# foamdino/incubator-druid

Measured on AMD Instinct MI355X. Metric: filtered rows aggregated/sec, higher is better.
Workload: dtype int64/f64; 1 GPU; BASELINE configs[2]: GroupByV2 dimUniform x dimHyperUnique (3-byte ids, ~1 group/row) + longSum/doubleSum, 100M rows = 8 x 12.5M-row segments per MI355X; config=groupby, segments_per_gpu=8, compression=lz4, lz4_mode=hc, bitmap=concise, long_encoding=longs, parallelism=segments sharded over 1 GPU(s)

## Files before the change

### incubator-druid_amd/csrc/dg_engine.cpp

```cpp
#include <hip/hip_runtime.h>

#include <algorithm>
#include <atomic>
#include <chrono>
#include <thread>
#include <functional>
#include <cerrno>
#include <cmath>
#include <cstdarg>
#include <cstdio>
#include <cstdlib>
#include <cstring>
#include <queue>
#include <unordered_map>
#include <string>
#include <string_view>
#include <vector>

#include "dg_internal.h"

namespace dg {

static thread_local char g_err[1024] = "";
static thread_local uint64_t g_err_count = 0;
// ... 4002 lines not shown
  if (choice.max_groups > 0) max_groups = std::min(max_groups, choice.max_groups);
  if (key_bits < 62) max_groups = std::min<int64_t>(max_groups, (int64_t)1 << key_bits);
  HashTable tab{};
  const bool use_hash = choice.grouper == DG_GROUPER_HASH && !has_float_sum(plan) && key_bits <= 63 &&
                        hash_capacity(max_groups) <= ((int64_t)1 << 31);
  if (use_hash) {
    tab.capacity = hash_capacity(max_groups);
    tab.log2_capacity = bits_for(tab.capacity);
    tab.max_groups = max_groups;
    tab.keys = dev_take<uint64_t>(cs, (size_t)tab.capacity);
    tab.slots = dev_take<uint64_t>(cs, (size_t)tab.capacity * rec);
    tab.ctr = dev_take<unsigned long long>(cs, 4);
    if (!tab.keys || !tab.slots || !tab.ctr)
      return set_error(DG_ERR_OOM, "hash table of %lld slots x %d words", (long long)tab.capacity, rec + 1);
    if (!call_err(cs, st)) return set_error(DG_ERR_OOM, "error word");
  }
  uint32_t* h_n = host_take<uint32_t>(cs, 4);
  if (!h_n) return set_error(DG_ERR_OOM, "groupBy counters");
  DG_FLUSH(cs, st);
  phase_event(ctx->ev[3], st);
  auto all_rows_in = [&](int i) {
    if (gj[i].bitset || gj[i].multi) return false;
    if (gj[i].time.kind == VIEW_ABSENT) return true;
    const Column* tc = sv[i]->find("__time");
    if (!tc || !tc->data.time_col || tc->data.nblocks <= 0 || tc->data.min8.size() != (size_t)tc->data.nblocks ||
        tc->data.max8.size() != (size_t)tc->data.nblocks)
      return false;
    const int64_t lo = *std::min_element(tc->data.min8.begin(), tc->data.min8.end());
    const int64_t hi = *std::max_element(tc->data.max8.begin(), tc->data.max8.end());
    return lo >= gj[i].t_lo && hi < gj[i].t_hi;
  };
  bool rows_elems = !any_multi && !has_float_sum(plan) && !env_on("DG_GB_COUNT");
  for (int i = 0; i < n && rows_elems; ++i) rows_elems = !cur[i].any || all_rows_in(i);
  launch_gb_keygen(d_jobs, d_tile, ntiles, &sb, plan, st, any_multi, rows_elems ? total : -1);
  phase_event(ctx->ev[5], st);
  unsigned long long* h_ctr = nullptr;
  if (use_hash) {
    h_ctr = host_take<unsigned long long>(cs, 4);
    if (!h_ctr) return set_error(DG_ERR_OOM, "groupBy counters");
    launch_gb_hash_fill(tab, plan, st);
    if (side) DG_HIP(hipStreamWaitEvent(st, ctx->side_ev[2], 0));
    launch_gb_hash_insert(&sb, sb.cap, tab, plan, cs->d_err, st);
    phase_event(ctx->ev[6], st);
    DG_HIP(hipMemcpyAsync(h_ctr, tab.ctr, 32, hipMemcpyDeviceToHost, st));
    DG_HIP(hipMemcpyAsync(h_n, sb.n, 4, hipMemcpyDeviceToHost, st));
    rc = finish_call(cs, st);
    if (rc == DG_ERR_TABLE_FULL)
      return set_error(DG_ERR_TABLE_FULL, "groupBy hash table full: more than %lld groups (bufferGrouperMaxSize; %lld slots)",
                       (long long)tab.max_groups, (long long)tab.capacity);
    if (rc) return rc;
  } else {
    launch_radix_sort(&sb, key_bits, st);
    phase_event(ctx->ev[6], st);
  }
  DG_CHECK_INTERRUPT(intr);
  const int64_t cap = std::max<int64_t>(use_hash ? (int64_t)h_ctr[0] : sb.cap, 1);
  PendingResult res(new dg_result());
  res->ctx = ctx;
  res->ndims = nd;
  res->naggs = na;
  res->lay = lay;
  res->bucket0 = gb0;
  res->period = q->period_ms;
  if (gr.hb) res->bounds.assign(gr.hb, gr.hb + gr.nb + 1);
  res->universal = q->interval_start;
  res->kinds.assign(plan.kind, plan.kind + na);
  res->dicts = md;
  res->keys = static_cast<uint64_t*>(result_alloc(ctx, (size_t)cap * 8));
  res->slots = static_cast<uint64_t*>(result_alloc(ctx, (size_t)cap * rec * 8));
  res->cap = cap;
  if (!res->keys || !res->slots) return set_error(DG_ERR_OOM, "groupBy result of %lld records", (long long)cap);
  bool reduce_timed = false;
  if (use_hash) {
    const int64_t ngh = (int64_t)h_ctr[0];
    phase_event(ctx->ev[7], st);
    reduce_timed = true;
    if (ngh > 0) {
      SortBufs gsb;
      rc = sort_bufs(cs, ngh, 1, key_bits, 0, &gsb, tab.log2_capacity);
      if (rc) return rc;
      launch_gb_hash_collect(tab, &gsb, ngh, st);
      launch_radix_sort(&gsb, key_bits, st);
      launch_gb_hash_emit(&gsb, ngh, tab, plan, res->keys, res->slots, cap, st);
    }
    res->grouper.grouper = DG_GROUPER_HASH;
// ... 37 lines not shown
        DG_HIP(hipStreamSynchronize(st));
        DG_HIP(hipGetLastError());
      }
      result_free(ctx, res->keys);
      result_free(ctx, res->slots);
      res->keys = k2;
      res->slots = s2;
      res->cap = c2;
    } else {
      result_free(ctx, k2);
      result_free(ctx, s2);
    }
  }
  if (side) {
    float fs = 0;
    phase_elapsed(&fs, ctx->side_ev[1], ctx->side_ev[2]);
    m.decode_side_ms = fs;
  }
  for (int i = 0; i < n; ++i)
    if (cur[i].any) m.pre_filtered_rows += counts[i] ? (int64_t)*counts[i] : sv[i]->nrows;
  m.selected_rows = nsel;
  float f1 = 0, f2 = 0, f3 = 0, f4 = 0, f5 = 0, f6 = 0;
  phase_elapsed(&f1, ctx->ev[0], ctx->ev[1]);
  phase_elapsed(&f2, ctx->ev[1], ctx->ev[2]);
  phase_elapsed(&f3, ctx->ev[3], ctx->ev[4]);
  phase_elapsed(&f4, ctx->ev[3], ctx->ev[5]);
  phase_elapsed(&f5, ctx->ev[5], ctx->ev[6]);
  phase_elapsed(&f6, ctx->ev[6], ctx->ev[4]);
  m.bitmap_ms = f1;
  m.bitmap_bytes = cs->bitmap_bytes;
  m.decode_ms = f2;
  decode_metrics(db, db_side, &m, ctx->ev[0]);
  m.aggregate_ms = f3;
  m.keygen_ms = f4;
  m.sort_ms = f5;
  m.reduce_ms = f6;
  if (reduce_timed) {
    float fr = 0;
    phase_elapsed(&fr, ctx->ev[7], ctx->ev[4]);
    m.reduce_kernel_ms = fr;
  }
  m.sort_passes = key_bits > 0 ? (key_bits + 7) / 8 : 0;
  m.key_bits = key_bits;
  m.groups = ng;
  m.total_ms = ms_since(t0);
  if (metrics) *metrics = m;
  *out = res.release();
  return DG_OK;
}

int64_t dg_result_groups(const dg_result* r) { return r ? r->ngroups : -1; }

int dg_result_grouper_info(const dg_result* r, dg_grouper_info* out) {
  if (!r || !out) return set_error(DG_ERR_ARG, "null argument");
  *out = r->grouper;
  return DG_OK;
}

int dg_result_fetch_groups(dg_result* r, int64_t start, int64_t count, int64_t* bucket_time, int32_t* ids,
                           uint64_t* values) {
  if (!r || start < 0 || count < 0 || start + count > r->ngroups) return set_error(DG_ERR_ARG, "bad result range");
  if (count == 0) return DG_OK;
  CallGuard g(r->ctx);
  CallScratch* cs = g.cs;
  hipStream_t st = r->ctx->stream;
  const int nd = r->ndims, na = r->naggs;
  const int64_t per = (bucket_time ? 8 : 0) + (ids ? 4 * (int64_t)nd : 0) + (values ? 8 * (int64_t)na : 0);
// ... 1072 lines not shown
```

### incubator-druid_amd/csrc/dg_internal.h

```cpp
#pragma once

#include <hip/hip_runtime.h>
#include <stdint.h>
#include <string.h>

#include <algorithm>
#include <atomic>
#include <map>
#include <memory>
#include <mutex>
#include <string>
#include <vector>

#include "../../include/druidgpu.h"

namespace dg {

constexpr int kMaxAggs = 16;
constexpr int kBlockBytes = 65536;

enum Codec : int32_t { CODEC_LZF = 0x00, CODEC_LZ4 = 0x01, CODEC_UNCOMPRESSED = 0xFF, CODEC_NONE = 0xFE };

enum ViewKind : int32_t { VIEW_ABSENT = 0, VIEW_LONG = 1, VIEW_FLOAT = 2, VIEW_DOUBLE = 3, VIEW_IDS = 4 };

// ... 474 lines not shown
  int32_t dim_mode;
  const int32_t* rank;
  int32_t lo, hi;
  int32_t min_rank;
  int32_t pad;
};
constexpr int kSelBlock = 1024;
constexpr int kTopnOrderCap = 4096;
void launch_topn_select(const TopnSelJob* d_jobs, int njobs, int64_t max_card, int naggs, int metric, int metric_op,
                        int inverted, int threshold, hipStream_t s);

constexpr int kTileRows = 2048;

#ifndef DG_RS_DIGIT_BITS
#define DG_RS_DIGIT_BITS 8
#endif
constexpr int kMaxDigitBits = DG_RS_DIGIT_BITS;
constexpr int kMaxBins = 1 << kMaxDigitBits;
constexpr int kRsMaxPasses = 8;
constexpr int kSortTile = 4096;
#ifndef DG_RED_WAVES
#define DG_RED_WAVES 16
#endif
constexpr int kRedWaves = DG_RED_WAVES;
constexpr int kMaxCallSegs = 1024;
inline int sort_tiles(int64_t n) { return (int)std::max<int64_t>(1, (n + kSortTile - 1) / kSortTile); }
void launch_gb_count(const GbJob* d_jobs, const int32_t* d_tile_job, int ntiles, uint32_t* tile_cnt, uint32_t* total,
                     bool multi, hipStream_t s);
void launch_gb_count_total(const GbJob* d_jobs, const int32_t* d_tile_job, int ntiles, uint32_t* tile_cnt,
                           unsigned long long* total, hipStream_t s);
void launch_gb_keygen(const GbJob* d_jobs, const int32_t* d_tile_job, int ntiles, SortBufs* sb, AggPlan plan,
                      hipStream_t s, bool multi = false, int64_t all_rows = -1);
void launch_radix_sort(SortBufs* sb, int key_bits, hipStream_t s);
void launch_run_heads(SortBufs* sb, hipStream_t s);
void launch_run_mark(SortBufs* sb, uint32_t* head_pos, hipStream_t s);
void launch_gb_reduce(SortBufs* sb, AggPlan plan, uint64_t* out_keys, uint64_t* out_slots, int64_t cap,
                      uint32_t* head_pos, int64_t* carry_g, uint64_t* carry_slots, int64_t* open_g, hipStream_t s);
void launch_fsum_runs(const GbJob* d_jobs, int njobs, int ntiles, SortBufs* sb, AggPlan plan, int agg,
                      const uint32_t* head_pos, uint64_t* out_slots, int64_t cap, hipStream_t s, int desc = 0);
void launch_slots_finalize(uint64_t* slots, const uint32_t* n_ptr, int64_t cap, AggPlan plan, hipStream_t s);
void launch_soa_to_aos(const uint64_t* soa, int64_t cap, int64_t n, int rec, uint64_t* aos, hipStream_t s);
void launch_result_compact(const uint64_t* keys, const uint64_t* slots, int64_t cap, int64_t n, int rec, uint64_t* keys2,
                           uint64_t* slots2, hipStream_t s);
constexpr uint64_t kHashEmpty = ~0ull;
constexpr int32_t kErrTableFull = 8;
constexpr int kHashTile = 4096;
struct HashTable {
  uint64_t* keys;
  uint64_t* slots;
  int64_t capacity;
  int log2_capacity;
  int64_t max_groups;
  unsigned long long* ctr;
};
inline int64_t hash_capacity(int64_t max_groups) {
  int64_t c = 1;
  while (c * 7 < max_groups * 10) c <<= 1;
  return c;
}
struct GrouperChoice {
  int32_t grouper;
  int64_t max_groups;
};
inline GrouperChoice resolve_grouper(const dg_groupby_opts* opts, int32_t ctx_grouper, int64_t ctx_max_groups,
                                     const char* env) {
  GrouperChoice c{ctx_grouper, ctx_max_groups > 0 ? ctx_max_groups : 0};
// ... 47 lines not shown
```

### incubator-druid_amd/csrc/dg_sort.hip

```cpp
#include <hip/hip_runtime.h>
#include <cstring>

#include "dg_device.h"

namespace dg {

static bool zero_async(void* p, size_t n, hipStream_t s) {
  const hipError_t e = hipMemsetAsync(p, 0, n, s);
  if (e != hipSuccess) note_launch_error(e);
  return e == hipSuccess;
}

constexpr int kST = 256;
constexpr int kSPT = kSortTile / kST;
#ifndef DG_RS_TILE_MUL
#define DG_RS_TILE_MUL 1
#endif
#ifndef DG_RS_THREADS
#define DG_RS_THREADS 256
#endif
constexpr int kRsTile = kSortTile * DG_RS_TILE_MUL;
constexpr int kRsT = DG_RS_THREADS;
constexpr int kRsW = kRsT / 64;
constexpr int kRsSPT = kRsTile / kRsT;

template <int NT>
__device__ __forceinline__ uint64_t block_scan_u64(uint64_t v, uint64_t* total, uint64_t* s_tmp) {
  const int lane = threadIdx.x & 63, wave = threadIdx.x >> 6;
  uint64_t x = v;
#pragma unroll
  for (int o = 1; o < 64; o <<= 1) {
    const uint64_t y = __shfl_up(x, o, 64);
    if (lane >= o) x += y;
  }
// ... 25 lines not shown
    const int i = base + threadIdx.x;
    const uint32_t v = i < n ? a[i] : 0u;
    uint32_t t;
    const uint32_t ex = block_scan_u32<1024>(v, &t, s_tmp);
    if (i < n) a[i] = carry + ex;
    carry += t;
  }
  if (threadIdx.x == 0) *total = carry;
}

__device__ __forceinline__ size_t pay_at(int pw, size_t i, int a) { return i * (size_t)pw + (size_t)a; }

__device__ __forceinline__ int locate_seg(const uint32_t* s_base, int njobs, uint32_t ref) {
  int lo = 0, hi = njobs - 1;
  while (lo < hi) {
    const int mid = (lo + hi + 1) >> 1;
    if (s_base[mid] <= ref) lo = mid;
    else hi = mid - 1;
  }
  return lo;
}

__device__ __forceinline__ bool gb_select(const GbJob& j, int64_t r, int64_t* bucket) {
  if (j.bitset && !((j.bitset[r >> 5] >> (r & 31)) & 1u)) return false;
  *bucket = 0;
  if (j.time.kind != VIEW_ABSENT) {
    const int64_t t = load_time(j.time, r);
    if (t < j.t_lo || t >= j.t_hi) return false;
    if (j.period) *bucket = (bucket_coord(j.bounds, j.nbounds, t) - j.bucket0) / j.period;
  }
  return true;
}

__device__ __forceinline__ uint64_t gb_key(const GbJob& j, int64_t r, int64_t bucket) {
  uint64_t k = ((uint64_t)j.seg_slot << j.seg_shift) | ((uint64_t)bucket << j.bucket_shift);
  for (int d = 0; d < j.ndims; ++d) {
    uint32_t g;
    if (j.dims[d].kind == VIEW_IDS) {
      const uint32_t id = load_id(j.dims[d], r);
      g = j.remap[d] ? (uint32_t)j.remap[d][id] : id;
    } else {
      g = (uint32_t)j.null_gid[d];
    }
    k |= (uint64_t)g << j.dim_shift[d];
  }
  return k;
}

__device__ __forceinline__ uint32_t gb_fanout(const GbJob& j, int64_t r) {
  uint64_t n = 1;
  for (int d = 0; d < j.ndims; ++d)
    if (j.moff[d].kind != VIEW_ABSENT) {
      const uint32_t a = load_id(j.moff[d], r), b = load_id(j.moff[d], r + 1);
      n *= b > a ? (uint64_t)(b - a) : (j.skip_empty ? 0ull : 1ull);
      n = n > 0xFFFFFFFFull ? 0xFFFFFFFFull : n;
    }
  return (uint32_t)n;
}

__device__ __forceinline__ uint64_t gb_key_multi(const GbJob& j, int64_t r, int64_t bucket, uint32_t c) {
  uint64_t k = ((uint64_t)j.seg_slot << j.seg_shift) | ((uint64_t)bucket << j.bucket_shift);
  for (int d = j.ndims - 1; d >= 0; --d) {
    uint32_t g = (uint32_t)j.null_gid[d];
    if (j.moff[d].kind != VIEW_ABSENT) {
      const uint32_t a = load_id(j.moff[d], r), b = load_id(j.moff[d], r + 1);
      if (b > a) {
        const uint32_t m = b - a, i = c % m;
        c /= m;
        const uint32_t id = load_id(j.dims[d], (int64_t)a + i);
        g = j.remap[d] ? (uint32_t)j.remap[d][id] : id;
      }
    } else if (j.dims[d].kind == VIEW_IDS) {
      const uint32_t id = load_id(j.dims[d], r);
      g = j.remap[d] ? (uint32_t)j.remap[d][id] : id;
    }
    k |= (uint64_t)g << j.dim_shift[d];
  }
  return k;
}
// ... 23 lines not shown

__global__ __launch_bounds__(1024) void k_sum_u64(const uint32_t* __restrict__ a, int n, unsigned long long* __restrict__ total) {
  __shared__ unsigned long long s[16];
  unsigned long long c = 0;
  for (int i = threadIdx.x; i < n; i += 1024) c += a[i];
  for (int o = 32; o > 0; o >>= 1) c += __shfl_down(c, o, 64);
  if ((threadIdx.x & 63) == 0) s[threadIdx.x >> 6] = c;
  __syncthreads();
  if (threadIdx.x == 0) {
    unsigned long long t = 0;
    for (int w = 0; w < 16; ++w) t += s[w];
    *total = t;
  }
}

void launch_gb_count_total(const GbJob* d_jobs, const int32_t* d_tile_job, int ntiles, uint32_t* tile_cnt,
                           unsigned long long* total, hipStream_t s) {
  if (ntiles <= 0) {
    zero_async(total, 8, s);
    return;
  }
  hipLaunchKernelGGL(k_gb_count<true>, dim3(ntiles), dim3(256), 0, s, d_jobs, d_tile_job, tile_cnt);
  hipLaunchKernelGGL(k_sum_u64, dim3(1), dim3(1024), 0, s, tile_cnt, ntiles, total);
}

__device__ __forceinline__ uint32_t elem_ref(uint64_t w, const uint32_t* refs, int64_t i, int kshift) {
  return refs ? refs[i] : (uint32_t)(w & ((1ull << kshift) - 1ull));
}

template <bool MULTI>
__global__ __launch_bounds__(256) void k_gb_keygen(const GbJob* __restrict__ jobs, const int32_t* __restrict__ tile_job,
                                                   const uint32_t* __restrict__ offs, uint64_t* __restrict__ keys,
                                                   uint32_t* __restrict__ refs, int kshift, AggPlan plan,
                                                   uint64_t* __restrict__ payload, int pw, int rowref, int rows_elems) {
  __shared__ uint32_t s_tmp[4];
  const GbJob& j = jobs[tile_job[blockIdx.x]];
  const int64_t r0 = (int64_t)(blockIdx.x - j.tile_begin) * kTileRows;
  const int64_t r1 = min((int64_t)j.nrows, r0 + kTileRows);
  uint32_t base = rows_elems ? j.row_base + (uint32_t)r0 : offs[blockIdx.x];
  const uint32_t inplace = rowref ? j.inplace : 0u;
  const bool all_inplace = pw > 0 && inplace == (pw >= 32 ? 0xFFFFFFFFu : (1u << pw) - 1u);
  auto emit = [&](uint32_t idx, uint32_t ref, uint64_t key, auto&& val) {
    if (refs) {
      keys[idx] = key;
      refs[idx] = ref;
    } else {
      keys[idx] = (key << kshift) | ref;
    }
    if (all_inplace) return;
    if (pw == 2 && !inplace) {
      *reinterpret_cast<ulonglong2*>(payload + (size_t)ref * 2) = make_ulonglong2(val(0), val(1));
    } else {
      for (int a = 0; a < pw; ++a)
        if (!((inplace >> a) & 1u)) payload[pay_at(pw, ref, a)] = val(a);
    }
  };
  bool all_rows = !MULTI && !j.bitset;
  int64_t tbucket = 0;
  if (all_rows && j.time.kind != VIEW_ABSENT) {
    const int64_t tk = r0 >> j.time.log2_per;
    all_rows = (reinterpret_cast<uintptr_t>(j.time.blocks[tk]) & 1u) && tk == ((r1 - 1) >> j.time.log2_per);
    if (all_rows) all_rows = gb_select(j, r0, &tbucket);
  }
  if (all_rows) {
    bool direct = pw <= kMaxAggs;
    for (int d = 0; d < j.ndims; ++d)
      direct &= j.dims[d].kind != VIEW_IDS ||
                (!(j.dims[d].pad & kViewBigEndian) && (r0 >> j.dims[d].log2_per) == ((r1 - 1) >> j.dims[d].log2_per));
    for (int a = 0; a < pw; ++a)
      direct &= ((inplace >> a) & 1u) || j.vals[a].kind == VIEW_ABSENT ||
                (r0 >> j.vals[a].log2_per) == ((r1 - 1) >> j.vals[a].log2_per);
    if (direct) {
      constexpr int kB = kTileRows / 256;
      static_assert(kTileRows % 256 == 0, "whole batches per tile");
      uint64_t key[kB];
#pragma unroll
      for (int u = 0; u < kB; ++u) key[u] = ((uint64_t)j.seg_slot << j.seg_shift) | ((uint64_t)tbucket << j.bucket_shift);
      auto load_ids = [&](int d, uint32_t* id) {
        const ColView& v = j.dims[d];
        if (v.kind != VIEW_IDS) return;
        const int64_t blk = r0 >> v.log2_per;
        const uint8_t* bp = v.blocks[blk];
#pragma unroll
        for (int u = 0; u < kB; ++u) {
          const int64_t r = r0 + threadIdx.x + 256 * u;
          id[u] = 0;
          if (r < r1) {
            const uint32_t off = (uint32_t)(r - (blk << v.log2_per)) * (uint32_t)v.width;
            if (v.width == 3) {
              const uint32_t* w = reinterpret_cast<const uint32_t*>(bp + (off & ~3u));
              id[u] = __builtin_amdgcn_alignbyte(w[1], w[0], off & 3u) & 0xFFFFFFu;
            } else if (v.width == 1) {
              id[u] = bp[off];
            } else if (v.width == 2) {
              id[u] = *reinterpret_cast<const uint16_t*>(bp + off);
            } else {
              id[u] = *reinterpret_cast<const uint32_t*>(bp + off);
            }
          }
        }
      };
      auto merge_ids = [&](int d, uint32_t* id) {
        const int32_t* rm = j.remap[d];
        if (j.dims[d].kind != VIEW_IDS) {
#pragma unroll
          for (int u = 0; u < kB; ++u) key[u] |= (uint64_t)(uint32_t)j.null_gid[d] << j.dim_shift[d];
          return;
        }
#pragma unroll
        for (int u = 0; u < kB; ++u) key[u] |= (uint64_t)(rm ? (uint32_t)rm[id[u]] : id[u]) << j.dim_shift[d];
      };
      if (j.ndims == 2) {
        uint32_t id0[kB], id1[kB];
        load_ids(0, id0);
        load_ids(1, id1);
        merge_ids(0, id0);
        merge_ids(1, id1);
      } else {
        for (int d = 0; d < j.ndims; ++d) {
          uint32_t id[kB];
          load_ids(d, id);
          merge_ids(d, id);
        }
      }
#pragma unroll
      for (int u = 0; u < kB; ++u) {
        const int64_t r = r0 + threadIdx.x + 256 * u;
        if (r >= r1) continue;
        const uint32_t idx = base + (uint32_t)(r - r0);
        emit(idx, rowref ? j.row_base + (uint32_t)r : idx, key[u], [&](int a) -> uint64_t {
          const ColView& v = j.vals[a];
          if (!agg_row(j.agg_bits[a], r)) return identity_of(plan.op[a], plan.kind[a]);
          if (plan.kind[a] == DG_AGG_COUNT || v.kind == VIEW_ABSENT) return agg_input_at(plan.kind[a], v.kind, nullptr);
          const int64_t blk = r0 >> v.log2_per;
          return agg_input_at(plan.kind[a], v.kind, v.blocks[blk] + (size_t)(r - (blk << v.log2_per)) * (size_t)v.width);
        });
      }
      return;
    }
    for (int64_t r = r0 + threadIdx.x; r < r1; r += 256) {
      const uint32_t idx = base + (uint32_t)(r - r0);
      emit(idx, rowref ? j.row_base + (uint32_t)r : idx, gb_key(j, r, tbucket), [&](int a) { return agg_in(j, plan, a, r); });
    }
    return;
  }
  for (int64_t rb = r0; rb < r1; rb += 256) {
    const int64_t r = rb + threadIdx.x;
    int64_t b = 0;
    const bool sel = r < r1 && gb_select(j, r, &b);
    uint32_t tot;
    if (MULTI) {
      const uint32_t nf = sel ? gb_fanout(j, r) : 0u;
      const uint32_t ex = block_scan_u32<256>(nf, &tot, s_tmp);
      for (uint32_t e = 0; e < nf; ++e)
        emit(base + ex + e, base + ex + e, gb_key_multi(j, r, b, e), [&](int a) { return agg_in(j, plan, a, r); });
      base += tot;
      continue;
// ... 2 lines not shown
    if (sel)
      emit(base + ex, rowref ? j.row_base + (uint32_t)r : base + ex, gb_key(j, r, b),
           [&](int a) { return agg_in(j, plan, a, r); });
    base += tot;
  }
}

void launch_gb_count(const GbJob* d_jobs, const int32_t* d_tile_job, int ntiles, uint32_t* tile_cnt, uint32_t* total,
                     bool multi, hipStream_t s) {
  if (ntiles <= 0) {
    zero_async(total, 4, s);
    return;
  }
  if (multi) hipLaunchKernelGGL(k_gb_count<true>, dim3(ntiles), dim3(256), 0, s, d_jobs, d_tile_job, tile_cnt);
  else hipLaunchKernelGGL(k_gb_count<false>, dim3(ntiles), dim3(256), 0, s, d_jobs, d_tile_job, tile_cnt);
  hipLaunchKernelGGL(k_scan_u32, dim3(1), dim3(1024), 0, s, tile_cnt, ntiles, total);
}

void launch_gb_keygen(const GbJob* d_jobs, const int32_t* d_tile_job, int ntiles, SortBufs* sb, AggPlan plan,
                      hipStream_t s, bool multi, int64_t all_rows) {
  if (ntiles <= 0) {
    zero_async(sb->n, 4, s);
    return;
  }
  const bool rows_elems = !multi && all_rows >= 0;
  if (rows_elems) {
    const hipError_t e = hipMemsetD32Async(reinterpret_cast<hipDeviceptr_t>(sb->n), (int)(uint32_t)all_rows, 1, s);
    if (e != hipSuccess) note_launch_error(e);
  } else {
    launch_gb_count(d_jobs, d_tile_job, ntiles, sb->tile_cnt, sb->n, multi, s);
  }
  if (multi)
    hipLaunchKernelGGL(k_gb_keygen<true>, dim3(ntiles), dim3(256), 0, s, d_jobs, d_tile_job, sb->tile_cnt,
                       sb->keys[sb->cur], sb->refs[sb->cur], sb->ref_bits, plan, sb->payload, sb->pw, 0, 0);
  else
    hipLaunchKernelGGL(k_gb_keygen<false>, dim3(ntiles), dim3(256), 0, s, d_jobs, d_tile_job, sb->tile_cnt,
                       sb->keys[sb->cur], sb->refs[sb->cur], sb->ref_bits, plan, sb->payload, sb->pw, sb->row_refs,
                       rows_elems ? 1 : 0);
}

template <class W>
struct Lb {
  static constexpr int kShift = 8 * sizeof(W) - 2;
  static constexpr W kAgg = (W)1 << kShift;
  static constexpr W kPre = (W)2 << kShift;
  static constexpr W kVal = ((W)1 << kShift) - 1;
};
constexpr uint64_t kLbAgg = Lb<uint64_t>::kAgg;
constexpr uint64_t kLbPre = Lb<uint64_t>::kPre;
constexpr uint64_t kLbVal = Lb<uint64_t>::kVal;

__global__ __launch_bounds__(kST) void k_rs_hist0(const uint64_t* __restrict__ keys, const uint32_t* __restrict__ n_ptr,
                                                  int shift, int bits, uint32_t* __restrict__ totals) {
  __shared__ uint32_t s_h[4][kMaxBins];
  const int tid = threadIdx.x, wave = tid >> 6;
  for (int i = tid; i < 4 * kMaxBins; i += kST) (&s_h[0][0])[i] = 0;
  __syncthreads();
  const uint32_t n = *n_ptr;
  const uint64_t mask = (1ull << bits) - 1;
  constexpr int kU = 4;
  const int64_t stride = (int64_t)gridDim.x * kST;
  int64_t i = (int64_t)blockIdx.x * kST + tid;
  for (; i + (kU - 1) * stride < (int64_t)n; i += kU * stride) {
    uint64_t w[kU];
#pragma unroll
    for (int u = 0; u < kU; ++u) w[u] = keys[i + u * stride];
#pragma unroll
    for (int u = 0; u < kU; ++u) atomicAdd(&s_h[wave][(int)((w[u] >> shift) & mask)], 1u);
  }
  for (; i < (int64_t)n; i += stride) atomicAdd(&s_h[wave][(int)((keys[i] >> shift) & mask)], 1u);
  __syncthreads();
  for (int d = tid; d < (1 << bits); d += kST) {
    const uint32_t c = s_h[0][d] + s_h[1][d] + s_h[2][d] + s_h[3][d];
    if (c) atomicAdd(&totals[d], c);
  }
}

__device__ __forceinline__ uint64_t match_digit(uint32_t d, int bits, bool valid) {
  uint64_t m = __ballot(valid);
  for (int b = 0; b < bits; ++b) {
    const bool x = (d >> b) & 1u;
    const uint64_t bb = __ballot(x);
    m &= x ? bb : ~bb;
  }
  return m;
}

__device__ __forceinline__ uint32_t lanes_below(uint64_t m) {
  return __builtin_amdgcn_mbcnt_hi((uint32_t)(m >> 32), __builtin_amdgcn_mbcnt_lo((uint32_t)m, 0u));
}

template <bool REFS, class W>
__global__ __launch_bounds__(kRsT) void k_rs_scatter(const uint64_t* __restrict__ kin, const uint32_t* __restrict__ vin,
                                                    uint64_t* __restrict__ kout, uint32_t* __restrict__ vout,
                                                    const uint32_t* __restrict__ n_ptr, int shift, int bits,
                                                    const uint32_t* __restrict__ totals, W* __restrict__ status,
                                                    uint32_t* __restrict__ tile_ctr, int nshift, int nbits,
                                                    uint32_t* __restrict__ ntotals) {
  __shared__ uint64_t s_k[kRsTile];
  __shared__ uint32_t s_v[REFS ? kRsTile : 1];
  __shared__ uint32_t s_cnt[kRsW * kMaxBins];
  __shared__ uint32_t s_next[kMaxBins];
  __shared__ int64_t s_delta[kMaxBins];
  __shared__ uint64_t s_tmp64[kRsW];
  __shared__ int s_tile;
  const int tid = threadIdx.x, lane = tid & 63, wave = tid >> 6;
  const uint32_t n = *n_ptr;
  if (tid == 0) s_tile = (int)atomicAdd(tile_ctr, 1u);
  uint64_t* s_peer = reinterpret_cast<uint64_t*>(s_k);
  static_assert(kRsW * kMaxBins <= kRsTile, "peer masks fit the tile buffer");
  for (int i = tid; i < kRsW * kMaxBins; i += kRsT) {
    s_cnt[i] = 0;
    s_peer[i] = 0;
  }
  for (int i = tid; i < kMaxBins; i += kRsT) s_next[i] = 0;
  __syncthreads();
  const int tile = s_tile;
  const int64_t base = (int64_t)tile * kRsTile;
  if (base >= n) return;
  const int tile_n = (int)min<int64_t>(kRsTile, (int64_t)n - base);
  const int nb = 1 << bits;
  const uint64_t dmask = (uint64_t)(nb - 1);
  const uint64_t nmask = (1ull << nbits) - 1;
  const int wbase = wave * (kRsTile / kRsW);
  uint64_t k[kRsSPT];
  uint32_t v[kRsSPT], rank[kRsSPT];
#pragma unroll
  for (int c = 0; c < kRsSPT; ++c) {
    const int x = wbase + c * 64 + lane;
    const bool ok = x < tile_n;
    k[c] = ok ? kin[base + x] : 0ull;
    if (REFS) v[c] = ok ? vin[base + x] : 0u;
  }
  uint32_t* cnt = s_cnt + wave * kMaxBins;
  uint64_t* peer = s_peer + wave * kMaxBins;
#pragma unroll
  for (int c = 0; c < kRsSPT; ++c) {
    const bool ok = wbase + c * 64 + lane < tile_n;
    const uint32_t d = (uint32_t)((k[c] >> shift) & dmask);
    if (ok) __hip_atomic_fetch_or(peer + d, 1ull << lane, __ATOMIC_RELAXED, __HIP_MEMORY_SCOPE_WORKGROUP);
    uint64_t peers = 0;
    uint32_t prior = 0;
    if (ok) {
      peers = peer[d];
      prior = cnt[d];
    }
    rank[c] = prior + lanes_below(peers);
    if (ok && 63 - __clzll((long long)peers) == lane) {
      cnt[d] = prior + (uint32_t)__popcll(peers);
      peer[d] = 0;
    }
  }
  __syncthreads();
  {
    constexpr int kDPT = kMaxBins > kRsT ? kMaxBins / kRsT : 1;
    static_assert(kMaxBins <= kRsT || kMaxBins % kRsT == 0, "digits per thread");
    uint32_t cw[kDPT][kRsW], ct[kDPT];
    uint64_t excl[kDPT];
    uint32_t csum = 0, gsum = 0;
#pragma unroll
    for (int j = 0; j < kDPT; ++j) {
      const int d = tid * kDPT + j;
      ct[j] = 0;
      excl[j] = 0;
#pragma unroll
// ... 59 lines not shown
        toff += ct[j];
        gex += totals[d];
      }
    }
  }
  __syncthreads();
#pragma unroll
  for (int c = 0; c < kRsSPT; ++c) {
    if (wbase + c * 64 + lane >= tile_n) continue;
    const uint32_t d = (uint32_t)((k[c] >> shift) & dmask);
    const uint32_t lp = cnt[d] + rank[c];
    s_k[lp] = k[c];
    if (REFS) s_v[lp] = v[c];
  }
  __syncthreads();
#pragma unroll
  for (int c = 0; c < kRsSPT; ++c) {
    const int i = c * kRsT + tid;
    if (i < tile_n) {
      const uint64_t kk = s_k[i];
      const int64_t pos = s_delta[(kk >> shift) & dmask] + i;
      kout[pos] = kk;
      if (REFS) vout[pos] = s_v[i];
      if (ntotals) atomicAdd(&s_next[(kk >> nshift) & nmask], 1u);
    }
  }
  if (ntotals) {
    __syncthreads();
    for (int dd = tid; dd < (1 << nbits); dd += kRsT)
      if (s_next[dd]) atomicAdd(&ntotals[dd], s_next[dd]);
  }
}

static void radix_passes(SortBufs* sb, int lo, int hi, hipStream_t s) {
  const int kb = hi - lo;
  if (kb <= 0) return;
  const int npass = (kb + kMaxDigitBits - 1) / kMaxDigitBits;
  const int w = (kb + npass - 1) / npass;
  const int nt = (sb->ntiles_sort + DG_RS_TILE_MUL - 1) / DG_RS_TILE_MUL;
  uint32_t* totals = sb->bin_total;
  uint32_t* ctr = sb->bin_total + kRsMaxPasses * kMaxBins;
  if (!zero_async(sb->bin_total, ((size_t)kRsMaxPasses * kMaxBins + kRsMaxPasses) * sizeof(uint32_t), s)) return;
  hipLaunchKernelGGL(k_rs_hist0, dim3(std::min(nt, 4096)), dim3(kST), 0, s, sb->keys[sb->cur], sb->n,
                     sb->ref_bits + lo, std::min(kb, w), totals);
  for (int p = 0, off = lo; p < npass; ++p, off += w) {
    const int bits = std::min(w, hi - off);
    const int shift = sb->ref_bits + off;
    const int nbits = p + 1 < npass ? std::min(w, hi - off - w) : 0;
    uint32_t* nt_tot = p + 1 < npass ? totals + (size_t)(p + 1) * kMaxBins : nullptr;
    const int in = sb->cur, out = sb->cur ^ 1;
    const char* wide = getenv("DG_SORT_WIDE_STATUS");
    const bool narrow = sb->cap < ((int64_t)1 << 30) && !(wide && *wide && *wide != '0');
    if (!zero_async(sb->lb_status, (size_t)(1 << bits) * nt * (narrow ? 4 : 8), s)) return;
    uint32_t* st32 = reinterpret_cast<uint32_t*>(sb->lb_status);
    uint64_t* st64 = sb->lb_status;
    const uint32_t* tp = totals + (size_t)p * kMaxBins;
    if (sb->refs[in] && narrow)
      hipLaunchKernelGGL((k_rs_scatter<true, uint32_t>), dim3(nt), dim3(kRsT), 0, s, sb->keys[in], sb->refs[in], sb->keys[out],
                         sb->refs[out], sb->n, shift, bits, tp, st32, ctr + p, shift + w, nbits, nt_tot);
    else if (sb->refs[in])
      hipLaunchKernelGGL((k_rs_scatter<true, uint64_t>), dim3(nt), dim3(kRsT), 0, s, sb->keys[in], sb->refs[in], sb->keys[out],
                         sb->refs[out], sb->n, shift, bits, tp, st64, ctr + p, shift + w, nbits, nt_tot);
    else if (narrow)
      hipLaunchKernelGGL((k_rs_scatter<false, uint32_t>), dim3(nt), dim3(kRsT), 0, s, sb->keys[in], nullptr, sb->keys[out],
                         nullptr, sb->n, shift, bits, tp, st32, ctr + p, shift + w, nbits, nt_tot);
    else
      hipLaunchKernelGGL((k_rs_scatter<false, uint64_t>), dim3(nt), dim3(kRsT), 0, s, sb->keys[in], nullptr, sb->keys[out],
                         nullptr, sb->n, shift, bits, tp, st64, ctr + p, shift + w, nbits, nt_tot);
    sb->cur = out;
  }
}

void launch_radix_sort(SortBufs* sb, int key_bits, hipStream_t s) {
  if (key_bits <= 0) return;
  static_assert(64 / kMaxDigitBits <= kRsMaxPasses, "passes of a 64-bit key");
  radix_passes(sb, 0, key_bits, s);
}

__global__ void k_probe_sort_fill(uint64_t* __restrict__ keys, int64_t n, int ref_bits) {
  for (int64_t i = (int64_t)blockIdx.x * blockDim.x + threadIdx.x; i < n; i += (int64_t)gridDim.x * blockDim.x) {
    uint64_t z = (uint64_t)i + 0x9E3779B97F4A7C15ull;
    z = (z ^ (z >> 30)) * 0xBF58476D1CE4E5B9ull;
    z = (z ^ (z >> 27)) * 0x94D049BB133111EBull;
    z ^= z >> 31;
    const uint64_t key = (((z & 0xFFFFFFFFull) % 100000ull) << 17) | ((z >> 32) % 100000ull);
    keys[i] = (key << ref_bits) | (uint64_t)i;
  }
}
__global__ void k_probe_sort_check(const uint64_t* __restrict__ keys, int64_t n, uint32_t* __restrict__ bad) {
  for (int64_t i = (int64_t)blockIdx.x * blockDim.x + threadIdx.x; i + 1 < n; i += (int64_t)gridDim.x * blockDim.x)
    if (keys[i] >= keys[i + 1]) atomicAdd(bad, 1u);
}

int probe_sort(int64_t n, int iters, double* ms, hipStream_t st) {
  if (n <= 0 || n >= (1ll << 30)) return set_error(DG_ERR_ARG, "probe: sort of %lld elements", (long long)n);
  SortBufs sb;
  memset(&sb, 0, sizeof sb);
  sb.cap = n;
  sb.ntiles_sort = sort_tiles(n);
  int rb = 1;
  while ((1ll << rb) < n) ++rb;
  sb.ref_bits = rb;
  const int key_bits = 34;
  void* mem[5] = {nullptr, nullptr, nullptr, nullptr, nullptr};
  const size_t sz[5] = {((size_t)n + 16) * 8, ((size_t)n + 16) * 8, (size_t)kMaxBins * sb.ntiles_sort * 8,
                        ((size_t)kMaxBins * kRsMaxPasses + kRsMaxPasses + 1) * 4, 16};
  int rc = DG_OK;
  for (int i = 0; i < 5 && rc == DG_OK; ++i)
    if (hipMalloc(&mem[i], sz[i]) != hipSuccess) rc = set_error(DG_ERR_OOM, "probe: sort buffers of %lld", (long long)n);
// ... 672 lines not shown
```

Measured before the change: 10.55 billion rows/s.

## Fuse groupBy key generation into radix sort histogram and first scatter pass

Result: faster. 10.83 billion rows/s, median of 6 (+2.7%).

```diff
diff --git a/incubator-druid_amd/csrc/dg_engine.cpp b/incubator-druid_amd/csrc/dg_engine.cpp
--- a/incubator-druid_amd/csrc/dg_engine.cpp
+++ b/incubator-druid_amd/csrc/dg_engine.cpp
@@ -4058,7 +4058,28 @@
   };
   bool rows_elems = !any_multi && !has_float_sum(plan) && !env_on("DG_GB_COUNT");
   for (int i = 0; i < n && rows_elems; ++i) rows_elems = !cur[i].any || all_rows_in(i);
-  launch_gb_keygen(d_jobs, d_tile, ntiles, &sb, plan, st, any_multi, rows_elems ? total : -1);
+  bool fused_keygen = rows_elems && !use_hash && ntiles > 0 && radix_sort_generates(&sb, key_bits, total) &&
+                      !env_on("DG_NO_FUSED_KEYGEN");
+  const uint32_t all_inplace = na >= 32 ? 0xFFFFFFFFu : (1u << na) - 1u;
+  int64_t keygen_rows = 0;
+  for (int i = 0; i < n && fused_keygen; ++i) {
+    if (!cur[i].any) continue;
+    const GbJob& j = gj[i];
+    fused_keygen = j.time.kind == VIEW_ABSENT;
+    if (j.inplace != all_inplace) keygen_rows += rows[i];
+    for (int d = 0; d < nd && fused_keygen; ++d)
+      fused_keygen = j.moff[d].kind == VIEW_ABSENT &&
+                     (j.dims[d].kind == VIEW_ABSENT || (j.dims[d].kind == VIEW_IDS && !(j.dims[d].pad & kViewBigEndian) &&
+                                                        j.dims[d].log2_per >= kRsGenMinBlockLog2));
+  }
+  fused_keygen = fused_keygen && keygen_rows * 4 <= total;
+  if (!fused_keygen) {
+    launch_gb_keygen(d_jobs, d_tile, ntiles, &sb, plan, st, any_multi, rows_elems ? total : -1);
+  } else if (keygen_rows > 0) {
+    for (int i = 0; i < n; ++i)
+      if (cur[i].any && gj[i].inplace != all_inplace)
+        launch_gb_keygen_payload(d_jobs, d_tile, gj[i].tile_begin, (int)((rows[i] + kTileRows - 1) / kTileRows), &sb, plan, st);
+  }
   phase_event(ctx->ev[5], st);
   unsigned long long* h_ctr = nullptr;
   if (use_hash) {
@@ -4076,7 +4097,8 @@
                        (long long)tab.max_groups, (long long)tab.capacity);
     if (rc) return rc;
   } else {
-    launch_radix_sort(&sb, key_bits, st);
+    if (fused_keygen) launch_gb_sort_generated(d_jobs, n, total, &sb, key_bits, st);
+    else launch_radix_sort(&sb, key_bits, st);
     phase_event(ctx->ev[6], st);
   }
   DG_CHECK_INTERRUPT(intr);
@@ -4180,7 +4202,7 @@
   m.decode_ms = f2;
   decode_metrics(db, db_side, &m, ctx->ev[0]);
   m.aggregate_ms = f3;
-  m.keygen_ms = f4;
+  m.keygen_ms = fused_keygen ? 0.0 : f4;
   m.sort_ms = f5;
   m.reduce_ms = f6;
   if (reduce_timed) {
diff --git a/incubator-druid_amd/csrc/dg_internal.h b/incubator-druid_amd/csrc/dg_internal.h
--- a/incubator-druid_amd/csrc/dg_internal.h
+++ b/incubator-druid_amd/csrc/dg_internal.h
@@ -530,6 +530,11 @@
 void launch_gb_keygen(const GbJob* d_jobs, const int32_t* d_tile_job, int ntiles, SortBufs* sb, AggPlan plan,
                       hipStream_t s, bool multi = false, int64_t all_rows = -1);
 void launch_radix_sort(SortBufs* sb, int key_bits, hipStream_t s);
+constexpr int kRsGenMinBlockLog2 = 13;
+bool radix_sort_generates(const SortBufs* sb, int key_bits, int64_t rows);
+void launch_gb_keygen_payload(const GbJob* d_jobs, const int32_t* d_tile_job, int tile0, int ntiles, SortBufs* sb,
+                              AggPlan plan, hipStream_t s);
+void launch_gb_sort_generated(const GbJob* d_jobs, int njobs, int64_t rows, SortBufs* sb, int key_bits, hipStream_t s);
 void launch_run_heads(SortBufs* sb, hipStream_t s);
 void launch_run_mark(SortBufs* sb, uint32_t* head_pos, hipStream_t s);
 void launch_gb_reduce(SortBufs* sb, AggPlan plan, uint64_t* out_keys, uint64_t* out_slots, int64_t cap,
diff --git a/incubator-druid_amd/csrc/dg_sort.hip b/incubator-druid_amd/csrc/dg_sort.hip
--- a/incubator-druid_amd/csrc/dg_sort.hip
+++ b/incubator-druid_amd/csrc/dg_sort.hip
@@ -1,5 +1,6 @@
 #include <hip/hip_runtime.h>
 #include <cstring>
+#include <type_traits>
 
 #include "dg_device.h"
 
@@ -91,19 +92,101 @@
   return true;
 }
 
+__device__ __forceinline__ uint64_t gb_key_base(const GbJob& j, int64_t bucket) {
+  return ((uint64_t)j.seg_slot << j.seg_shift) | ((uint64_t)bucket << j.bucket_shift);
+}
+
+__device__ __forceinline__ uint64_t gb_dim_field(const GbJob& j, int d, uint32_t id) {
+  uint32_t g;
+  if (j.dims[d].kind == VIEW_IDS) g = j.remap[d] ? (uint32_t)j.remap[d][id] : id;
+  else g = (uint32_t)j.null_gid[d];
+  return (uint64_t)g << j.dim_shift[d];
+}
+
+__device__ __forceinline__ uint64_t gb_pack(uint64_t key, int kshift, uint32_t ref) { return (key << kshift) | ref; }
+
 __device__ __forceinline__ uint64_t gb_key(const GbJob& j, int64_t r, int64_t bucket) {
-  uint64_t k = ((uint64_t)j.seg_slot << j.seg_shift) | ((uint64_t)bucket << j.bucket_shift);
-  for (int d = 0; d < j.ndims; ++d) {
-    uint32_t g;
-    if (j.dims[d].kind == VIEW_IDS) {
-      const uint32_t id = load_id(j.dims[d], r);
-      g = j.remap[d] ? (uint32_t)j.remap[d][id] : id;
+  uint64_t k = gb_key_base(j, bucket);
+  for (int d = 0; d < j.ndims; ++d) k |= gb_dim_field(j, d, j.dims[d].kind == VIEW_IDS ? load_id(j.dims[d], r) : 0u);
+  return k;
+}
+
+template <int W>
+__device__ __forceinline__ uint32_t gb_block_id(const uint8_t* bp, uint32_t row) {
+  const uint32_t off = row * (uint32_t)W;
+  if (W == 3) {
+    const uint32_t* w = reinterpret_cast<const uint32_t*>(bp + (off & ~3u));
+    return __builtin_amdgcn_alignbyte(w[1], w[0], off & 3u) & 0xFFFFFFu;
+  }
+  if (W == 1) return bp[off];
+  if (W == 2) return *reinterpret_cast<const uint16_t*>(bp + off);
+  return *reinterpret_cast<const uint32_t*>(bp + off);
+}
+
+struct GbBlocks {
+  int64_t ba;
+  const uint8_t* pa;
+  const uint8_t* pb;
+};
+template <int kB, class Rows>
+__device__ __forceinline__ void gb_batch_keys(const GbJob& j, int64_t bucket, const Rows& rows, uint64_t* key,
+                                              uint64_t need = ~0ull) {
+#pragma unroll
+  for (int u = 0; u < kB; ++u) key[u] = gb_key_base(j, bucket);
+  auto needed = [&](int d) {
+    const uint64_t field = (j.dim_bits[d] >= 64 ? 0ull : 1ull << j.dim_bits[d]) - 1ull;
+    return ((field << j.dim_shift[d]) & need) != 0;
+  };
+  auto load_ids = [&](int d, uint32_t* id) {
+    const ColView& v = j.dims[d];
+#pragma unroll
+    for (int u = 0; u < kB; ++u) id[u] = 0;
+    if (v.kind != VIEW_IDS || !needed(d)) return;
+    const GbBlocks b = rows.blocks(v);
+    const int log2_per = v.log2_per;
+    const int64_t in_block = ((int64_t)1 << log2_per) - 1;
+    auto load_w = [&](auto w) {
+#pragma unroll
+      for (int u = 0; u < kB; ++u) {
+        const int64_t r = rows.row(u);
+        id[u] = gb_block_id<decltype(w)::value>((r >> log2_per) == b.ba ? b.pa : b.pb, (uint32_t)(r & in_block));
+      }
+    };
+    switch (v.width) {
+      case 1: load_w(std::integral_constant<int, 1>()); break;
+      case 2: load_w(std::integral_constant<int, 2>()); break;
+      case 3: load_w(std::integral_constant<int, 3>()); break;
+      default: load_w(std::integral_constant<int, 4>()); break;
+    }
+  };
+  auto merge_ids = [&](int d, const uint32_t* id) {
+    const int32_t* rm = j.remap[d];
+    const int sh = j.dim_shift[d];
+    if (!needed(d)) return;
+    if (j.dims[d].kind != VIEW_IDS) {
+#pragma unroll
+      for (int u = 0; u < kB; ++u) key[u] |= (uint64_t)(uint32_t)j.null_gid[d] << sh;
+    } else if (rm) {
+#pragma unroll
+      for (int u = 0; u < kB; ++u) key[u] |= (uint64_t)(uint32_t)rm[id[u]] << sh;
     } else {
-      g = (uint32_t)j.null_gid[d];
-    }
-    k |= (uint64_t)g << j.dim_shift[d];
-  }
-  return k;
+#pragma unroll
+      for (int u = 0; u < kB; ++u) key[u] |= (uint64_t)id[u] << sh;
+    }
+  };
+  if (j.ndims == 2) {
+    uint32_t id0[kB], id1[kB];
+    load_ids(0, id0);
+    load_ids(1, id1);
+    merge_ids(0, id0);
+    merge_ids(1, id1);
+  } else {
+    for (int d = 0; d < j.ndims; ++d) {
+      uint32_t id[kB];
+      load_ids(d, id);
+      merge_ids(d, id);
+    }
+  }
 }
 
 __device__ __forceinline__ uint32_t gb_fanout(const GbJob& j, int64_t r) {
@@ -193,20 +276,23 @@
 __global__ __launch_bounds__(256) void k_gb_keygen(const GbJob* __restrict__ jobs, const int32_t* __restrict__ tile_job,
                                                    const uint32_t* __restrict__ offs, uint64_t* __restrict__ keys,
                                                    uint32_t* __restrict__ refs, int kshift, AggPlan plan,
-                                                   uint64_t* __restrict__ payload, int pw, int rowref, int rows_elems) {
+                                                   uint64_t* __restrict__ payload, int pw, int rowref, int rows_elems,
+                                                   int tile0) {
   __shared__ uint32_t s_tmp[4];
-  const GbJob& j = jobs[tile_job[blockIdx.x]];
-  const int64_t r0 = (int64_t)(blockIdx.x - j.tile_begin) * kTileRows;
+  const int tile = (int)blockIdx.x + tile0;
+  const GbJob& j = jobs[tile_job[tile]];
+  const int64_t r0 = (int64_t)(tile - j.tile_begin) * kTileRows;
   const int64_t r1 = min((int64_t)j.nrows, r0 + kTileRows);
-  uint32_t base = rows_elems ? j.row_base + (uint32_t)r0 : offs[blockIdx.x];
+  uint32_t base = rows_elems ? j.row_base + (uint32_t)r0 : offs[tile];
   const uint32_t inplace = rowref ? j.inplace : 0u;
   const bool all_inplace = pw > 0 && inplace == (pw >= 32 ? 0xFFFFFFFFu : (1u << pw) - 1u);
   auto emit = [&](uint32_t idx, uint32_t ref, uint64_t key, auto&& val) {
-    if (refs) {
+    if (!keys) {
+    } else if (refs) {
       keys[idx] = key;
       refs[idx] = ref;
     } else {
-      keys[idx] = (key << kshift) | ref;
+      keys[idx] = gb_pack(key, kshift, ref);
     }
     if (all_inplace) return;
     if (pw == 2 && !inplace) {
@@ -234,56 +320,17 @@
     if (direct) {
       constexpr int kB = kTileRows / 256;
       static_assert(kTileRows % 256 == 0, "whole batches per tile");
-      uint64_t key[kB];
-#pragma unroll
-      for (int u = 0; u < kB; ++u) key[u] = ((uint64_t)j.seg_slot << j.seg_shift) | ((uint64_t)tbucket << j.bucket_shift);
-      auto load_ids = [&](int d, uint32_t* id) {
-        const ColView& v = j.dims[d];
-        if (v.kind != VIEW_IDS) return;
-        const int64_t blk = r0 >> v.log2_per;
-        const uint8_t* bp = v.blocks[blk];
-#pragma unroll
-        for (int u = 0; u < kB; ++u) {
-          const int64_t r = r0 + threadIdx.x + 256 * u;
-          id[u] = 0;
-          if (r < r1) {
-            const uint32_t off = (uint32_t)(r - (blk << v.log2_per)) * (uint32_t)v.width;
-            if (v.width == 3) {
-              const uint32_t* w = reinterpret_cast<const uint32_t*>(bp + (off & ~3u));
-              id[u] = __builtin_amdgcn_alignbyte(w[1], w[0], off & 3u) & 0xFFFFFFu;
-            } else if (v.width == 1) {
-              id[u] = bp[off];
-            } else if (v.width == 2) {
-              id[u] = *reinterpret_cast<const uint16_t*>(bp + off);
-            } else {
-              id[u] = *reinterpret_cast<const uint32_t*>(bp + off);
-            }
-          }
+      struct TileRows {
+        int64_t r0, r1;
+        __device__ __forceinline__ int64_t row(int u) const { return min(r0 + threadIdx.x + 256 * u, r1 - 1); }
+        __device__ __forceinline__ GbBlocks blocks(const ColView& v) const {
+          const int64_t blk = r0 >> v.log2_per;
+          const uint8_t* bp = v.blocks[blk];
+          return GbBlocks{blk, bp, bp};
         }
       };
-      auto merge_ids = [&](int d, uint32_t* id) {
-        const int32_t* rm = j.remap[d];
-        if (j.dims[d].kind != VIEW_IDS) {
-#pragma unroll
-          for (int u = 0; u < kB; ++u) key[u] |= (uint64_t)(uint32_t)j.null_gid[d] << j.dim_shift[d];
-          return;
-        }
-#pragma unroll
-        for (int u = 0; u < kB; ++u) key[u] |= (uint64_t)(rm ? (uint32_t)rm[id[u]] : id[u]) << j.dim_shift[d];
-      };
-      if (j.ndims == 2) {
-        uint32_t id0[kB], id1[kB];
-        load_ids(0, id0);
-        load_ids(1, id1);
-        merge_ids(0, id0);
-        merge_ids(1, id1);
-      } else {
-        for (int d = 0; d < j.ndims; ++d) {
-          uint32_t id[kB];
-          load_ids(d, id);
-          merge_ids(d, id);
-        }
-      }
+      uint64_t key[kB];
+      gb_batch_keys<kB>(j, tbucket, TileRows{r0, r1}, key);
 #pragma unroll
       for (int u = 0; u < kB; ++u) {
         const int64_t r = r0 + threadIdx.x + 256 * u;
@@ -352,11 +399,18 @@
   }
   if (multi)
     hipLaunchKernelGGL(k_gb_keygen<true>, dim3(ntiles), dim3(256), 0, s, d_jobs, d_tile_job, sb->tile_cnt,
-                       sb->keys[sb->cur], sb->refs[sb->cur], sb->ref_bits, plan, sb->payload, sb->pw, 0, 0);
+                       sb->keys[sb->cur], sb->refs[sb->cur], sb->ref_bits, plan, sb->payload, sb->pw, 0, 0, 0);
   else
     hipLaunchKernelGGL(k_gb_keygen<false>, dim3(ntiles), dim3(256), 0, s, d_jobs, d_tile_job, sb->tile_cnt,
                        sb->keys[sb->cur], sb->refs[sb->cur], sb->ref_bits, plan, sb->payload, sb->pw, sb->row_refs,
-                       rows_elems ? 1 : 0);
+                       rows_elems ? 1 : 0, 0);
+}
+
+void launch_gb_keygen_payload(const GbJob* d_jobs, const int32_t* d_tile_job, int tile0, int ntiles, SortBufs* sb,
+                              AggPlan plan, hipStream_t s) {
+  if (ntiles <= 0) return;
+  hipLaunchKernelGGL(k_gb_keygen<false>, dim3(ntiles), dim3(256), 0, s, d_jobs, d_tile_job, sb->tile_cnt, nullptr, nullptr,
+                     sb->ref_bits, plan, sb->payload, sb->pw, sb->row_refs, 1, tile0);
 }
 
 template <class W>
@@ -370,25 +424,105 @@
 constexpr uint64_t kLbPre = Lb<uint64_t>::kPre;
 constexpr uint64_t kLbVal = Lb<uint64_t>::kVal;
 
+constexpr int kSrcWords = 0, kSrcGen = 1;
+#ifndef DG_RS_GEN_BATCH
+#define DG_RS_GEN_BATCH 4
+#endif
+#ifndef DG_RS_GEN_BATCH_HIST
+#define DG_RS_GEN_BATCH_HIST 8
+#endif
+struct RsGen {
+  const GbJob* jobs;
+  int njobs;
+  int kshift;
+};
+
+__device__ __forceinline__ int rs_gen_job(const RsGen& g, uint32_t e) {
+  int lo = 0, hi = g.njobs - 1;
+  while (lo < hi) {
+    const int mid = (lo + hi + 1) >> 1;
+    if (g.jobs[mid].row_base <= e) lo = mid;
+    else hi = mid - 1;
+  }
+  return lo;
+}
+
+template <int NC, int G>
+__device__ __forceinline__ void rs_gen_words(const RsGen& g, uint32_t e_wave, uint32_t e_end, int lane, uint64_t* k,
+                                             uint64_t need = ~0ull) {
+  static_assert(NC * 64 <= (1 << kRsGenMinBlockLog2), "a share spans at most two blocks of a view");
+  e_wave = (uint32_t)__builtin_amdgcn_readfirstlane((int)e_wave);
+  e_end = (uint32_t)__builtin_amdgcn_readfirstlane((int)e_end);
+#pragma unroll
+  for (int c = 0; c < NC; ++c) k[c] = 0;
+  if (e_wave >= e_end) return;
+  const uint32_t e_last = min(e_end, e_wave + (uint32_t)(NC * 64)) - 1u;
+  for (int ji = rs_gen_job(g, e_wave), jl = rs_gen_job(g, e_last); ji <= jl; ++ji) {
+    const GbJob& j = g.jobs[ji];
+    if (j.nrows <= 0) continue;
+    const uint32_t lo = max(e_wave, j.row_base), hi = min(e_last, j.row_base + (uint32_t)j.nrows - 1u);
+    if (lo > hi) continue;
+    struct ShareRows {
+      int64_t r_first;
+      int64_t r_lo, r_hi;
+      int lane;
+      __device__ __forceinline__ int64_t row(int u) const { return min(max(r_first + 64 * u + lane, r_lo), r_hi); }
+      __device__ __forceinline__ GbBlocks blocks(const ColView& v) const {
+        const int64_t ba = r_lo >> v.log2_per;
+        return GbBlocks{ba, v.blocks[ba], v.blocks[r_hi >> v.log2_per]};
+      }
+    };
+    constexpr int kG = NC < G ? NC : G;
+    static_assert(NC % kG == 0, "whole batches per share");
+#pragma unroll
+    for (int c0 = 0; c0 < NC; c0 += kG) {
+      if (e_wave + (uint32_t)(64 * c0) > hi || e_wave + (uint32_t)(64 * (c0 + kG) - 1) < lo) continue;
+      uint64_t key[kG];
+      gb_batch_keys<kG>(j, 0, ShareRows{(int64_t)e_wave + 64 * c0 - (int64_t)j.row_base, (int64_t)(lo - j.row_base),
+                                        (int64_t)(hi - j.row_base), lane}, key, need >> g.kshift);
+#pragma unroll
+      for (int c = 0; c < kG; ++c) {
+        const uint32_t e = e_wave + (uint32_t)(64 * (c0 + c) + lane);
+        if (e >= lo && e <= hi) k[c0 + c] = gb_pack(key[c], g.kshift, e);
+      }
+    }
+  }
+}
+
+template <int SRC>
 __global__ __launch_bounds__(kST) void k_rs_hist0(const uint64_t* __restrict__ keys, const uint32_t* __restrict__ n_ptr,
-                                                  int shift, int bits, uint32_t* __restrict__ totals) {
+                                                  int shift, int bits, uint32_t* __restrict__ totals, RsGen gen) {
   __shared__ uint32_t s_h[4][kMaxBins];
   const int tid = threadIdx.x, wave = tid >> 6;
   for (int i = tid; i < 4 * kMaxBins; i += kST) (&s_h[0][0])[i] = 0;
   __syncthreads();
   const uint32_t n = *n_ptr;
   const uint64_t mask = (1ull << bits) - 1;
-  constexpr int kU = 4;
-  const int64_t stride = (int64_t)gridDim.x * kST;
-  int64_t i = (int64_t)blockIdx.x * kST + tid;
-  for (; i + (kU - 1) * stride < (int64_t)n; i += kU * stride) {
-    uint64_t w[kU];
-#pragma unroll
-    for (int u = 0; u < kU; ++u) w[u] = keys[i + u * stride];
-#pragma unroll
-    for (int u = 0; u < kU; ++u) atomicAdd(&s_h[wave][(int)((w[u] >> shift) & mask)], 1u);
-  }
-  for (; i < (int64_t)n; i += stride) atomicAdd(&s_h[wave][(int)((keys[i] >> shift) & mask)], 1u);
+  if (SRC == kSrcGen) {
+    constexpr int kNC = kSortTile / kST;
+    const uint32_t wbase = (uint32_t)wave * (uint32_t)(kNC * 64);
+    for (int64_t base = (int64_t)blockIdx.x * kSortTile; base < (int64_t)n; base += (int64_t)gridDim.x * kSortTile) {
+      const uint32_t e_end = (uint32_t)min<int64_t>((int64_t)n, base + kSortTile);
+      const uint32_t e_wave = (uint32_t)base + wbase;
+      uint64_t w[kNC];
+      rs_gen_words<kNC, DG_RS_GEN_BATCH_HIST>(gen, e_wave, e_end, tid & 63, w, mask << shift);
+#pragma unroll
+      for (int c = 0; c < kNC; ++c)
+        if (e_wave + (uint32_t)(64 * c + (tid & 63)) < e_end) atomicAdd(&s_h[wave][(int)((w[c] >> shift) & mask)], 1u);
+    }
+  } else {
+    constexpr int kU = 4;
+    const int64_t stride = (int64_t)gridDim.x * kST;
+    int64_t i = (int64_t)blockIdx.x * kST + tid;
+    for (; i + (kU - 1) * stride < (int64_t)n; i += kU * stride) {
+      uint64_t w[kU];
+#pragma unroll
+      for (int u = 0; u < kU; ++u) w[u] = keys[i + u * stride];
+#pragma unroll
+      for (int u = 0; u < kU; ++u) atomicAdd(&s_h[wave][(int)((w[u] >> shift) & mask)], 1u);
+    }
+    for (; i < (int64_t)n; i += stride) atomicAdd(&s_h[wave][(int)((keys[i] >> shift) & mask)], 1u);
+  }
   __syncthreads();
   for (int d = tid; d < (1 << bits); d += kST) {
     const uint32_t c = s_h[0][d] + s_h[1][d] + s_h[2][d] + s_h[3][d];
@@ -410,13 +544,14 @@
   return __builtin_amdgcn_mbcnt_hi((uint32_t)(m >> 32), __builtin_amdgcn_mbcnt_lo((uint32_t)m, 0u));
 }
 
-template <bool REFS, class W>
+template <bool REFS, class W, int SRC>
 __global__ __launch_bounds__(kRsT) void k_rs_scatter(const uint64_t* __restrict__ kin, const uint32_t* __restrict__ vin,
                                                     uint64_t* __restrict__ kout, uint32_t* __restrict__ vout,
                                                     const uint32_t* __restrict__ n_ptr, int shift, int bits,
                                                     const uint32_t* __restrict__ totals, W* __restrict__ status,
                                                     uint32_t* __restrict__ tile_ctr, int nshift, int nbits,
-                                                    uint32_t* __restrict__ ntotals) {
+                                                    uint32_t* __restrict__ ntotals, RsGen gen) {
+  static_assert(SRC == kSrcWords || !REFS, "generated elements are packed words");
   __shared__ uint64_t s_k[kRsTile];
   __shared__ uint32_t s_v[REFS ? kRsTile : 1];
   __shared__ uint32_t s_cnt[kRsW * kMaxBins];
@@ -445,12 +580,16 @@
   const int wbase = wave * (kRsTile / kRsW);
   uint64_t k[kRsSPT];
   uint32_t v[kRsSPT], rank[kRsSPT];
-#pragma unroll
-  for (int c = 0; c < kRsSPT; ++c) {
-    const int x = wbase + c * 64 + lane;
-    const bool ok = x < tile_n;
-    k[c] = ok ? kin[base + x] : 0ull;
-    if (REFS) v[c] = ok ? vin[base + x] : 0u;
+  if (SRC == kSrcGen) {
+    rs_gen_words<kRsSPT, DG_RS_GEN_BATCH>(gen, (uint32_t)base + (uint32_t)wbase, (uint32_t)base + (uint32_t)tile_n, lane, k);
+  } else {
+#pragma unroll
+    for (int c = 0; c < kRsSPT; ++c) {
+      const int x = wbase + c * 64 + lane;
+      const bool ok = x < tile_n;
+      k[c] = ok ? kin[base + x] : 0ull;
+      if (REFS) v[c] = ok ? vin[base + x] : 0u;
+    }
   }
   uint32_t* cnt = s_cnt + wave * kMaxBins;
   uint64_t* peer = s_peer + wave * kMaxBins;
@@ -576,7 +715,7 @@
   }
 }
 
-static void radix_passes(SortBufs* sb, int lo, int hi, hipStream_t s) {
+static void radix_passes(SortBufs* sb, int lo, int hi, hipStream_t s, const RsGen* gen) {
   const int kb = hi - lo;
   if (kb <= 0) return;
   const int npass = (kb + kMaxDigitBits - 1) / kMaxDigitBits;
@@ -585,8 +724,13 @@
   uint32_t* totals = sb->bin_total;
   uint32_t* ctr = sb->bin_total + kRsMaxPasses * kMaxBins;
   if (!zero_async(sb->bin_total, ((size_t)kRsMaxPasses * kMaxBins + kRsMaxPasses) * sizeof(uint32_t), s)) return;
-  hipLaunchKernelGGL(k_rs_hist0, dim3(std::min(nt, 4096)), dim3(kST), 0, s, sb->keys[sb->cur], sb->n,
-                     sb->ref_bits + lo, std::min(kb, w), totals);
+  const RsGen none{nullptr, 0, 0};
+  if (gen)
+    hipLaunchKernelGGL(k_rs_hist0<kSrcGen>, dim3(std::min(nt, 4096)), dim3(kST), 0, s, nullptr, sb->n, sb->ref_bits + lo,
+                       std::min(kb, w), totals, *gen);
+  else
+    hipLaunchKernelGGL(k_rs_hist0<kSrcWords>, dim3(std::min(nt, 4096)), dim3(kST), 0, s, sb->keys[sb->cur], sb->n,
+                       sb->ref_bits + lo, std::min(kb, w), totals, none);
   for (int p = 0, off = lo; p < npass; ++p, off += w) {
     const int bits = std::min(w, hi - off);
     const int shift = sb->ref_bits + off;
@@ -599,18 +743,24 @@
     uint32_t* st32 = reinterpret_cast<uint32_t*>(sb->lb_status);
     uint64_t* st64 = sb->lb_status;
     const uint32_t* tp = totals + (size_t)p * kMaxBins;
-    if (sb->refs[in] && narrow)
-      hipLaunchKernelGGL((k_rs_scatter<true, uint32_t>), dim3(nt), dim3(kRsT), 0, s, sb->keys[in], sb->refs[in], sb->keys[out],
-                         sb->refs[out], sb->n, shift, bits, tp, st32, ctr + p, shift + w, nbits, nt_tot);
+    if (gen && p == 0 && narrow)
+      hipLaunchKernelGGL((k_rs_scatter<false, uint32_t, kSrcGen>), dim3(nt), dim3(kRsT), 0, s, nullptr, nullptr, sb->keys[out],
+                         nullptr, sb->n, shift, bits, tp, st32, ctr + p, shift + w, nbits, nt_tot, *gen);
+    else if (gen && p == 0)
+      hipLaunchKernelGGL((k_rs_scatter<false, uint64_t, kSrcGen>), dim3(nt), dim3(kRsT), 0, s, nullptr, nullptr, sb->keys[out],
+                         nullptr, sb->n, shift, bits, tp, st64, ctr + p, shift + w, nbits, nt_tot, *gen);
+    else if (sb->refs[in] && narrow)
+      hipLaunchKernelGGL((k_rs_scatter<true, uint32_t, kSrcWords>), dim3(nt), dim3(kRsT), 0, s, sb->keys[in], sb->refs[in],
+                         sb->keys[out], sb->refs[out], sb->n, shift, bits, tp, st32, ctr + p, shift + w, nbits, nt_tot, none);
     else if (sb->refs[in])
-      hipLaunchKernelGGL((k_rs_scatter<true, uint64_t>), dim3(nt), dim3(kRsT), 0, s, sb->keys[in], sb->refs[in], sb->keys[out],
-                         sb->refs[out], sb->n, shift, bits, tp, st64, ctr + p, shift + w, nbits, nt_tot);
+      hipLaunchKernelGGL((k_rs_scatter<true, uint64_t, kSrcWords>), dim3(nt), dim3(kRsT), 0, s, sb->keys[in], sb->refs[in],
+                         sb->keys[out], sb->refs[out], sb->n, shift, bits, tp, st64, ctr + p, shift + w, nbits, nt_tot, none);
     else if (narrow)
-      hipLaunchKernelGGL((k_rs_scatter<false, uint32_t>), dim3(nt), dim3(kRsT), 0, s, sb->keys[in], nullptr, sb->keys[out],
-                         nullptr, sb->n, shift, bits, tp, st32, ctr + p, shift + w, nbits, nt_tot);
+      hipLaunchKernelGGL((k_rs_scatter<false, uint32_t, kSrcWords>), dim3(nt), dim3(kRsT), 0, s, sb->keys[in], nullptr,
+                         sb->keys[out], nullptr, sb->n, shift, bits, tp, st32, ctr + p, shift + w, nbits, nt_tot, none);
     else
-      hipLaunchKernelGGL((k_rs_scatter<false, uint64_t>), dim3(nt), dim3(kRsT), 0, s, sb->keys[in], nullptr, sb->keys[out],
-                         nullptr, sb->n, shift, bits, tp, st64, ctr + p, shift + w, nbits, nt_tot);
+      hipLaunchKernelGGL((k_rs_scatter<false, uint64_t, kSrcWords>), dim3(nt), dim3(kRsT), 0, s, sb->keys[in], nullptr,
+                         sb->keys[out], nullptr, sb->n, shift, bits, tp, st64, ctr + p, shift + w, nbits, nt_tot, none);
     sb->cur = out;
   }
 }
@@ -618,7 +768,21 @@
 void launch_radix_sort(SortBufs* sb, int key_bits, hipStream_t s) {
   if (key_bits <= 0) return;
   static_assert(64 / kMaxDigitBits <= kRsMaxPasses, "passes of a 64-bit key");
-  radix_passes(sb, 0, key_bits, s);
+  radix_passes(sb, 0, key_bits, s, nullptr);
+}
+
+bool radix_sort_generates(const SortBufs* sb, int key_bits, int64_t rows) {
+  return key_bits > 0 && !sb->refs[0] && sb->row_refs && rows > 0 && rows <= (int64_t)0xFFFFFFFFll - kRsTile;
+}
+
+void launch_gb_sort_generated(const GbJob* d_jobs, int njobs, int64_t rows, SortBufs* sb, int key_bits, hipStream_t s) {
+  const hipError_t e = hipMemsetD32Async(reinterpret_cast<hipDeviceptr_t>(sb->n), (int)(uint32_t)rows, 1, s);
+  if (e != hipSuccess) {
+    note_launch_error(e);
+    return;
+  }
+  const RsGen gen{d_jobs, njobs, sb->ref_bits};
+  radix_passes(sb, 0, key_bits, s, &gen);
 }
 
 __global__ void k_probe_sort_fill(uint64_t* __restrict__ keys, int64_t n, int ref_bits) {
```
